# jkulhanek/viewformer

Measured on AMD Instinct MI355X. Metric: novel views/sec (encode->AR transformer->decode), 128px 6-ctx, higher is better.
Workload: dtype bf16

## Files before the change

viewformer_amd/csrc/conv_in_x3h.hip:

```cpp
#include "halo_common.h"

namespace {

typedef _Float16 f16x8 __attribute__((ext_vector_type(8)));
typedef _Float16 f16x4 __attribute__((ext_vector_type(4)));

constexpr int TH = 8, TW = 16, BN = 128;
constexpr int PW = TW + 2, PH = TH + 2, NPIX = PH * PW;
constexpr int P_LDB = 16;
constexpr int PLANE_BYTES = 2 * BN * 16;
constexpr int KS_BYTES = 2 * PLANE_BYTES;
constexpr int BLK_BYTES = 3 * KS_BYTES;
constexpr int TAIL_BYTES = 16;

__device__ __forceinline__ void split2(float x, _Float16& h, _Float16& l) {
    h = (_Float16)x;
    l = (_Float16)((x - (float)h) * 2048.f);
}

template <bool U8>
__global__ __launch_bounds__(256) void conv_in_x3h_kernel(vf_igemm_args p, const unsigned char* __restrict__ img_u8) {
    __shared__ __attribute__((aligned(16))) unsigned char patch[NPIX * P_LDB];
    const int tid = threadIdx.x;
    const int lane = tid & 63;
    const int wave = __builtin_amdgcn_readfirstlane(tid >> 6);
    const int wave_m = wave >> 1, wave_n = wave & 1;
    const int half = lane >> 5, l31 = lane & 31;

    const int nb = p.Cout / BN;
    const int tilesX = p.Wout / TW, tilesY = p.Hout / TH;
    int bid = (int)vf_xcd_bid();
    const int nblk = bid % nb; bid /= nb;
    const int tx = bid % tilesX; bid /= tilesX;
    const int ty = bid % tilesY;
    const int img = bid / tilesY;
    const int y0 = ty * TH, x0 = tx * TW;

    if (tid < NPIX) {
        const int pr = tid / PW, pc = tid - pr * PW;
        const int sy = y0 - 1 + pr, sx = x0 - 1 + pc;
        const bool ok = sy >= 0 && sy < p.Hout && sx >= 0 && sx < p.Wout;
        const size_t px = ((size_t)img * p.Hout + (ok ? sy : 0)) * p.Wout + (ok ? sx : 0);
        f16x4 oh, ol;
#pragma unroll
        for (int c = 0; c < 3; ++c) {
            float v;
            if (U8) v = ((float)img_u8[px * 3 + c] * (1.0f / 255.0f)) * 2.0f - 1.0f;
            else v = p.x[px * 3 + c];
            _Float16 h, l;
            split2(ok ? v : 0.f, h, l);
            oh[c] = h; ol[c] = l;
        }
        oh[3] = (_Float16)0.f; ol[3] = (_Float16)0.f;
        *reinterpret_cast<f16x4*>(patch + tid * P_LDB) = oh;
        *reinterpret_cast<f16x4*>(patch + tid * P_LDB + 8) = ol;
    }

    const unsigned char* __restrict__ Wb = reinterpret_cast<const unsigned char*>(p.w_packed) + (size_t)nblk * BLK_BYTES +
                                           (half * BN + wave_n * 64 + l31) * 16;
    f16x8 b[3][2][2];
#pragma unroll
    for (int ks = 0; ks < 3; ++ks)
#pragma unroll
        for (int pl = 0; pl < 2; ++pl)
#pragma unroll
            for (int j = 0; j < 2; ++j) b[ks][pl][j] = *reinterpret_cast<const f16x8*>(Wb + ks * KS_BYTES + pl * PLANE_BYTES + j * 32 * 16);

    f32x16 acc[2][2], accx[2][2];
#pragma unroll
    for (int i = 0; i < 2; ++i)
#pragma unroll
        for (int j = 0; j < 2; ++j)
#pragma unroll
            for (int r = 0; r < 16; ++r) { acc[i][j][r] = 0.f; accx[i][j][r] = 0.f; }
    __syncthreads();

    const int trow = vf_perm_row(l31), tpx = vf_perm_px(l31);
#pragma unroll
    for (int ks = 0; ks < 3; ++ks) {
        const int g = ks * 2 + half;
        f16x8 a[2][2];
#pragma unroll
        for (int mi = 0; mi < 2; ++mi) {
            const int a0 = wave_m * 4 + mi * 2 + trow;
#pragma unroll
            for (int pl = 0; pl < 2; ++pl) {
                f16x4 lo = {(_Float16)0.f, (_Float16)0.f, (_Float16)0.f, (_Float16)0.f}, hi = lo;
                const int t0 = 2 * g, t1 = 2 * g + 1;
                if (t0 < 9) lo = *reinterpret_cast<const f16x4*>(patch + ((a0 + t0 / 3) * PW + tpx + t0 % 3) * P_LDB + pl * 8);
                if (t1 < 9) hi = *reinterpret_cast<const f16x4*>(patch + ((a0 + t1 / 3) * PW + tpx + t1 % 3) * P_LDB + pl * 8);
                a[mi][pl] = f16x8{lo[0], lo[1], lo[2], lo[3], hi[0], hi[1], hi[2], hi[3]};
            }
        }
#pragma unroll
        for (int mi = 0; mi < 2; ++mi)
#pragma unroll
            for (int j = 0; j < 2; ++j) accx[mi][j] = __builtin_amdgcn_mfma_f32_32x32x16_f16(a[mi][1], b[ks][0][j], accx[mi][j], 0, 0, 0);
#pragma unroll
        for (int mi = 0; mi < 2; ++mi)
#pragma unroll
            for (int j = 0; j < 2; ++j) accx[mi][j] = __builtin_amdgcn_mfma_f32_32x32x16_f16(a[mi][0], b[ks][1][j], accx[mi][j], 0, 0, 0);
#pragma unroll
        for (int mi = 0; mi < 2; ++mi)
#pragma unroll
            for (int j = 0; j < 2; ++j) acc[mi][j] = __builtin_amdgcn_mfma_f32_32x32x16_f16(a[mi][0], b[ks][0][j], acc[mi][j], 0, 0, 0);
    }

    const float inv_s = *reinterpret_cast<const float*>(reinterpret_cast<const unsigned char*>(p.w_packed) + (size_t)nb * BLK_BYTES);
#pragma unroll
    for (int i = 0; i < 2; ++i)
#pragma unroll
        for (int j = 0; j < 2; ++j)
#pragma unroll
            for (int r = 0; r < 16; ++r) acc[i][j][r] = __builtin_fmaf(accx[i][j][r], 4.8828125e-4f, acc[i][j][r]) * inv_s;
    vf_halo_epilogue<false>(p, acc, img, img, y0, x0, (ty * tilesX + tx) * 2, nblk, wave_m, wave_n, half, l31);
}

__global__ void absmax27_kernel(const float* __restrict__ w, long long n, unsigned* __restrict__ out) {
    float m = 0.f;
    for (long long i = blockIdx.x * (long long)blockDim.x + threadIdx.x; i < n; i += (long long)gridDim.x * blockDim.x) m = fmaxf(m, fabsf(w[i]));
    vf_block_max_atomic(m, out);
}

__global__ void pack_conv_in_x3h_kernel(const float* __restrict__ w, _Float16* __restrict__ dst, int Cout, int nb,
                                        unsigned char* __restrict__ tail) {
    const float amax = __uint_as_float(*reinterpret_cast<const unsigned*>(tail + 4));
    const int ex = amax > 0.f ? ilogbf(amax) : 13;
    const float S = ldexpf(1.f, 13 - ex);
    if (blockIdx.x == 0 && threadIdx.x == 0) *reinterpret_cast<float*>(tail) = ldexpf(1.f, ex - 13);
    const int total = nb * 3 * 2 * BN * 8;
    for (int idx = blockIdx.x * blockDim.x + threadIdx.x; idx < total; idx += gridDim.x * blockDim.x) {
        const int e = idx & 7;
        int t = idx >> 3;
        const int nl = t % BN; t /= BN;
        const int half = t & 1;
        const int ks = (t >> 1) % 3;
        const int nblk = (t >> 1) / 3;
        const int k = (ks * 2 + half) * 8 + e;
        const int tap = k >> 2, c = k & 3;
        const int n = nblk * BN + nl;
        float v = 0.f;
        if (tap < 9 && c < 3 && n < Cout) v = w[((size_t)n * 3 + c) * 9 + tap] * S;
        _Float16 h, l;
        split2(v, h, l);
        const size_t base = (((size_t)nblk * 3 + ks) * 2) * (2 * BN * 8) + ((size_t)half * BN + nl) * 8 + e;
        dst[base] = h;
        dst[base + 2 * BN * 8] = l;
    }
}

}

extern "C" {

size_t vf_conv_in_x3h_packed_elems(int Cout) {
    if (Cout <= 0 || Cout % BN) return 0;
    return (size_t)(Cout / BN) * 3 * 2 * 2 * BN * 8 + TAIL_BYTES / 2;
}

int vf_conv_in_x3h_pack(const float* w_oihw, void* dst, int Cout, void* stream) {
    if (!w_oihw || !dst || Cout <= 0) return VF_ERR_BAD_ARG;
    if (Cout % BN) return VF_ERR_UNSUPPORTED;
    const int nb = Cout / BN;
    unsigned char* tail = reinterpret_cast<unsigned char*>(dst) + (size_t)nb * BLK_BYTES;
    hipStream_t s = (hipStream_t)stream;
    if (hipMemsetAsync(tail, 0, TAIL_BYTES, s) != hipSuccess) return vf_last_status();
    hipLaunchKernelGGL(absmax27_kernel, dim3(16), dim3(256), 0, s, w_oihw, (long long)Cout * 27, reinterpret_cast<unsigned*>(tail + 4));
    hipLaunchKernelGGL(pack_conv_in_x3h_kernel, dim3(48), dim3(256), 0, s, w_oihw, (_Float16*)dst, Cout, nb, tail);
    return vf_last_status();
}

int vf_conv_in_x3h(const uint8_t* img_u8, const float* img_f32, const void* w_packed, const float* bias, float* out, float* gn_part,
                   int gn_slots, int n_img, int H, int W, int Cout, void* stream) {
    if ((!img_u8 && !img_f32) || !w_packed || !out || n_img <= 0 || H <= 0 || W <= 0 || Cout <= 0) return VF_ERR_BAD_ARG;
    if (H % TH || W % TW || Cout % BN) return VF_ERR_UNSUPPORTED;
    vf_igemm_args a = {};
    a.x = img_f32;
    a.w_packed = reinterpret_cast<const float*>(w_packed);
    a.bias = bias;
    a.out = out;
    a.mode = VF_MODE_CONV3_S1;
    a.M = n_img * H * W; a.Cin = 3; a.Cout = Cout;
    a.Hin = a.Hout = H; a.Win = a.Wout = W;
    a.lda = 3; a.ldc = Cout; a.ldr = Cout;
    a.batch = 1;
    a.gn_part = gn_part;
    a.gn_slots = gn_slots;
    if (int st = vf_halo_gn_check(a)) return st;
    const long long blocks = (long long)n_img * (H / TH) * (W / TW) * (Cout / BN);
    if (img_u8) hipLaunchKernelGGL(conv_in_x3h_kernel<true>, dim3((unsigned)blocks), dim3(256), 0, (hipStream_t)stream, a, img_u8);
    else hipLaunchKernelGGL(conv_in_x3h_kernel<false>, dim3((unsigned)blocks), dim3(256), 0, (hipStream_t)stream, a, img_u8);
    return vf_last_status();
}

}
```

Before: 1137.

## Make conv_in blocks persistent across a tile row with LDS weights and double-buffered patches

Each block now sweeps every horizontal tile of its tile row instead of handling a single tile. The block's weight slice is staged once into LDS. The next tile's input pixels are loaded and split into fp16 hi/lo while the current tile's MFMAs and epilogue run, using two patch buffers. The goal is to amortise the weight loads and launch overhead and to hide image-load latency. In exchange the grid shrinks by a factor of W/TW, which lowers parallelism for this small first conv and adds a per-tile barrier.

```diff
diff --git a/viewformer_amd/csrc/conv_in_x3h.hip b/viewformer_amd/csrc/conv_in_x3h.hip
--- a/viewformer_amd/csrc/conv_in_x3h.hip
+++ b/viewformer_amd/csrc/conv_in_x3h.hip
@@ -19,8 +19,9 @@
 }
 
 template <bool U8>
-__global__ __launch_bounds__(256) void conv_in_x3h_kernel(vf_igemm_args p, const unsigned char* __restrict__ img_u8) {
-    __shared__ __attribute__((aligned(16))) unsigned char patch[NPIX * P_LDB];
+__global__ __launch_bounds__(256, 2) void conv_in_x3h_kernel(vf_igemm_args p, const unsigned char* __restrict__ img_u8) {
+    __shared__ __attribute__((aligned(16))) unsigned char patch2[2][NPIX * P_LDB];
+    __shared__ __attribute__((aligned(16))) unsigned char wlds[BLK_BYTES];
     const int tid = threadIdx.x;
     const int lane = tid & 63;
     const int wave = __builtin_amdgcn_readfirstlane(tid >> 6);
@@ -31,89 +32,112 @@
     const int tilesX = p.Wout / TW, tilesY = p.Hout / TH;
     int bid = (int)vf_xcd_bid();
     const int nblk = bid % nb; bid /= nb;
-    const int tx = bid % tilesX; bid /= tilesX;
     const int ty = bid % tilesY;
     const int img = bid / tilesY;
-    const int y0 = ty * TH, x0 = tx * TW;
-
-    if (tid < NPIX) {
-        const int pr = tid / PW, pc = tid - pr * PW;
-        const int sy = y0 - 1 + pr, sx = x0 - 1 + pc;
-        const bool ok = sy >= 0 && sy < p.Hout && sx >= 0 && sx < p.Wout;
-        const size_t px = ((size_t)img * p.Hout + (ok ? sy : 0)) * p.Wout + (ok ? sx : 0);
-        f16x4 oh, ol;
-#pragma unroll
-        for (int c = 0; c < 3; ++c) {
-            float v;
-            if (U8) v = ((float)img_u8[px * 3 + c] * (1.0f / 255.0f)) * 2.0f - 1.0f;
-            else v = p.x[px * 3 + c];
-            _Float16 h, l;
-            split2(ok ? v : 0.f, h, l);
-            oh[c] = h; ol[c] = l;
-        }
-        oh[3] = (_Float16)0.f; ol[3] = (_Float16)0.f;
-        *reinterpret_cast<f16x4*>(patch + tid * P_LDB) = oh;
-        *reinterpret_cast<f16x4*>(patch + tid * P_LDB + 8) = ol;
-    }
-
-    const unsigned char* __restrict__ Wb = reinterpret_cast<const unsigned char*>(p.w_packed) + (size_t)nblk * BLK_BYTES +
-                                           (half * BN + wave_n * 64 + l31) * 16;
-    f16x8 b[3][2][2];
-#pragma unroll
-    for (int ks = 0; ks < 3; ++ks)
-#pragma unroll
-        for (int pl = 0; pl < 2; ++pl)
-#pragma unroll
-            for (int j = 0; j < 2; ++j) b[ks][pl][j] = *reinterpret_cast<const f16x8*>(Wb + ks * KS_BYTES + pl * PLANE_BYTES + j * 32 * 16);
-
-    f32x16 acc[2][2], accx[2][2];
-#pragma unroll
-    for (int i = 0; i < 2; ++i)
-#pragma unroll
-        for (int j = 0; j < 2; ++j)
-#pragma unroll
-            for (int r = 0; r < 16; ++r) { acc[i][j][r] = 0.f; accx[i][j][r] = 0.f; }
-    __syncthreads();
-
-    const int trow = vf_perm_row(l31), tpx = vf_perm_px(l31);
-#pragma unroll
-    for (int ks = 0; ks < 3; ++ks) {
-        const int g = ks * 2 + half;
-        f16x8 a[2][2];
-#pragma unroll
-        for (int mi = 0; mi < 2; ++mi) {
-            const int a0 = wave_m * 4 + mi * 2 + trow;
-#pragma unroll
-            for (int pl = 0; pl < 2; ++pl) {
-                f16x4 lo = {(_Float16)0.f, (_Float16)0.f, (_Float16)0.f, (_Float16)0.f}, hi = lo;
-                const int t0 = 2 * g, t1 = 2 * g + 1;
-                if (t0 < 9) lo = *reinterpret_cast<const f16x4*>(patch + ((a0 + t0 / 3) * PW + tpx + t0 % 3) * P_LDB + pl * 8);
-                if (t1 < 9) hi = *reinterpret_cast<const f16x4*>(patch + ((a0 + t1 / 3) * PW + tpx + t1 % 3) * P_LDB + pl * 8);
-                a[mi][pl] = f16x8{lo[0], lo[1], lo[2], lo[3], hi[0], hi[1], hi[2], hi[3]};
+    const int y0 = ty * TH;
+
+    const int pr = tid / PW, pc = tid - pr * PW;
+    const int sy = y0 - 1 + pr;
+    const bool row_ok = tid < NPIX && sy >= 0 && sy < p.Hout;
+    const size_t row_px = ((size_t)img * p.Hout + (row_ok ? sy : 0)) * p.Wout;
+    float raw[3];
+    auto load_raw = [&](int x0) {
+        const int sx = x0 - 1 + pc;
+        const bool ok = row_ok && sx >= 0 && sx < p.Wout;
+        const size_t px = ok ? row_px + sx : row_px;
+        if (tid < NPIX) {
+#pragma unroll
+            for (int c = 0; c < 3; ++c) {
+                float v;
+                if (U8) v = ((float)img_u8[px * 3 + c] * (1.0f / 255.0f)) * 2.0f - 1.0f;
+                else v = p.x[px * 3 + c];
+                raw[c] = ok ? v : 0.f;
             }
         }
-#pragma unroll
-        for (int mi = 0; mi < 2; ++mi)
-#pragma unroll
-            for (int j = 0; j < 2; ++j) accx[mi][j] = __builtin_amdgcn_mfma_f32_32x32x16_f16(a[mi][1], b[ks][0][j], accx[mi][j], 0, 0, 0);
-#pragma unroll
-        for (int mi = 0; mi < 2; ++mi)
-#pragma unroll
-            for (int j = 0; j < 2; ++j) accx[mi][j] = __builtin_amdgcn_mfma_f32_32x32x16_f16(a[mi][0], b[ks][1][j], accx[mi][j], 0, 0, 0);
-#pragma unroll
-        for (int mi = 0; mi < 2; ++mi)
-#pragma unroll
-            for (int j = 0; j < 2; ++j) acc[mi][j] = __builtin_amdgcn_mfma_f32_32x32x16_f16(a[mi][0], b[ks][0][j], acc[mi][j], 0, 0, 0);
+    };
+    auto park = [&](unsigned char* patch) {
+        if (tid < NPIX) {
+            f16x4 oh, ol;
+#pragma unroll
+            for (int c = 0; c < 3; ++c) {
+                _Float16 h, l;
+                split2(raw[c], h, l);
+                oh[c] = h; ol[c] = l;
+            }
+            oh[3] = (_Float16)0.f; ol[3] = (_Float16)0.f;
+            *reinterpret_cast<f16x4*>(patch + tid * P_LDB) = oh;
+            *reinterpret_cast<f16x4*>(patch + tid * P_LDB + 8) = ol;
+        }
+    };
+    load_raw(0);
+
+    {
+        const f32x4* __restrict__ src = reinterpret_cast<const f32x4*>(reinterpret_cast<const unsigned char*>(p.w_packed) + (size_t)nblk * BLK_BYTES);
+#pragma unroll
+        for (int i = 0; i < BLK_BYTES / 16 / 256; ++i) reinterpret_cast<f32x4*>(wlds)[tid + i * 256] = src[tid + i * 256];
     }
-
+    const unsigned char* Wb = wlds + (half * BN + wave_n * 64 + l31) * 16;
     const float inv_s = *reinterpret_cast<const float*>(reinterpret_cast<const unsigned char*>(p.w_packed) + (size_t)nb * BLK_BYTES);
-#pragma unroll
-    for (int i = 0; i < 2; ++i)
-#pragma unroll
-        for (int j = 0; j < 2; ++j)
-#pragma unroll
-            for (int r = 0; r < 16; ++r) acc[i][j][r] = __builtin_fmaf(accx[i][j][r], 4.8828125e-4f, acc[i][j][r]) * inv_s;
-    vf_halo_epilogue<false>(p, acc, img, img, y0, x0, (ty * tilesX + tx) * 2, nblk, wave_m, wave_n, half, l31);
+
+    park(patch2[0]);
+    __syncthreads();
+
+    const int trow = vf_perm_row(l31), tpx = vf_perm_px(l31);
+    for (int tx = 0; tx < tilesX; ++tx) {
+        const unsigned char* patch = patch2[tx & 1];
+        const bool more = tx + 1 < tilesX;
+
+        f32x16 acc[2][2], accx[2][2];
+#pragma unroll
+        for (int i = 0; i < 2; ++i)
+#pragma unroll
+            for (int j = 0; j < 2; ++j)
+#pragma unroll
+                for (int r = 0; r < 16; ++r) { acc[i][j][r] = 0.f; accx[i][j][r] = 0.f; }
+#pragma unroll
+        for (int ks = 0; ks < 3; ++ks) {
+            const int g = ks * 2 + half;
+            f16x8 a[2][2], b[2][2];
+#pragma unroll
+            for (int pl = 0; pl < 2; ++pl)
+#pragma unroll
+                for (int j = 0; j < 2; ++j) b[pl][j] = *reinterpret_cast<const f16x8*>(Wb + ks * KS_BYTES + pl * PLANE_BYTES + j * 32 * 16);
+#pragma unroll
+            for (int mi = 0; mi < 2; ++mi) {
+                const int a0 = wave_m * 4 + mi * 2 + trow;
+#pragma unroll
+                for (int pl = 0; pl < 2; ++pl) {
+                    f16x4 lo = {(_Float16)0.f, (_Float16)0.f, (_Float16)0.f, (_Float16)0.f}, hi = lo;
+                    const int t0 = 2 * g, t1 = 2 * g + 1;
+                    if (t0 < 9) lo = *reinterpret_cast<const f16x4*>(patch + ((a0 + t0 / 3) * PW + tpx + t0 % 3) * P_LDB + pl * 8);
+                    if (t1 < 9) hi = *reinterpret_cast<const f16x4*>(patch + ((a0 + t1 / 3) * PW + tpx + t1 % 3) * P_LDB + pl * 8);
+                    a[mi][pl] = f16x8{lo[0], lo[1], lo[2], lo[3], hi[0], hi[1], hi[2], hi[3]};
+                }
+            }
+#pragma unroll
+            for (int mi = 0; mi < 2; ++mi)
+#pragma unroll
+                for (int j = 0; j < 2; ++j) accx[mi][j] = __builtin_amdgcn_mfma_f32_32x32x16_f16(a[mi][1], b[0][j], accx[mi][j], 0, 0, 0);
+#pragma unroll
+            for (int mi = 0; mi < 2; ++mi)
+#pragma unroll
+                for (int j = 0; j < 2; ++j) accx[mi][j] = __builtin_amdgcn_mfma_f32_32x32x16_f16(a[mi][0], b[1][j], accx[mi][j], 0, 0, 0);
+#pragma unroll
+            for (int mi = 0; mi < 2; ++mi)
+#pragma unroll
+                for (int j = 0; j < 2; ++j) acc[mi][j] = __builtin_amdgcn_mfma_f32_32x32x16_f16(a[mi][0], b[0][j], acc[mi][j], 0, 0, 0);
+        }
+        if (more) load_raw((tx + 1) * TW);
+#pragma unroll
+        for (int i = 0; i < 2; ++i)
+#pragma unroll
+            for (int j = 0; j < 2; ++j)
+#pragma unroll
+                for (int r = 0; r < 16; ++r) acc[i][j][r] = __builtin_fmaf(accx[i][j][r], 4.8828125e-4f, acc[i][j][r]) * inv_s;
+        if (more) park(patch2[(tx + 1) & 1]);
+        __syncthreads();
+        vf_halo_epilogue<false>(p, acc, img, img, y0, tx * TW, (ty * tilesX + tx) * 2, nblk, wave_m, wave_n, half, l31);
+    }
 }
 
 __global__ void absmax27_kernel(const float* __restrict__ w, long long n, unsigned* __restrict__ out) {
@@ -187,7 +211,7 @@
     a.gn_part = gn_part;
     a.gn_slots = gn_slots;
     if (int st = vf_halo_gn_check(a)) return st;
-    const long long blocks = (long long)n_img * (H / TH) * (W / TW) * (Cout / BN);
+    const long long blocks = (long long)n_img * (H / TH) * (Cout / BN);
     if (img_u8) hipLaunchKernelGGL(conv_in_x3h_kernel<true>, dim3((unsigned)blocks), dim3(256), 0, (hipStream_t)stream, a, img_u8);
     else hipLaunchKernelGGL(conv_in_x3h_kernel<false>, dim3((unsigned)blocks), dim3(256), 0, (hipStream_t)stream, a, img_u8);
     return vf_last_status();
```

Result: no change. 1139, median of 3 (+0.2%).
